# Alxaline/BraTS21

Hardware: AMD Instinct MI355X
Metric: train patches/sec (4x128^3, width-48) (higher is better)
Workload: dtype bf16; 1 GPU; equiunet width=48, batch=2/GPU of 4x128^3 synthetic patches, fwd + deep-supervision Dice + bwd + ranger (BASELINE.json configs[1]); global_batch=2, parallelism=dp1

## Files before the change

brats21_amd/csrc/conv_wgrad.hip:

```cpp
#include <stdlib.h>
#include "twin_begin.hpp"
#include "common.hpp"

typedef __attribute__((ext_vector_type(4))) short s16x4;

struct WgradParams {
  const void* x1; const void* x2; int c1, c2, p1, p2;
  const void* dy; int dyp;
  float* ws;
  int N, D, H, W, cin, cout;
  int tz, ty, tx, ntiles, nsplit;
  int nlane;
  int ntaps, dil;
  int seglen, nsegz;
};

constexpr int WG_TZ = 4, WG_TY = 4, WG_TX = 16, WG_VOX = 256;

template <typename T, int DIL, int COF, int CIF, int KS = 3>
struct WgGeom {
  static constexpr bool BF = std::is_same<T, bf16_t>::value;
  static constexpr int ESZ = sizeof(T);
  static constexpr int EPL = 16 / ESZ;
  static constexpr int R = KS == 3 ? DIL : 0;
  static constexpr int HY = WG_TY + 2 * R, HX = WG_TX + 2 * R;
  static constexpr int HVOX = WG_TZ * HY * HX;
  static constexpr int CI_T = 16 * CIF, CO_T = 16 * COF;
  static constexpr int XROWB = CI_T * ESZ, YROWB = CO_T * ESZ;
  static constexpr int SX = BF ? (CIF == 1 ? 32 : 96) : XROWB + 16;
  static constexpr int SY = BF ? (COF == 1 ? 32 : 96) : YROWB + 16;
  static constexpr int XPPV = XROWB / 16, YPPV = YROWB / 16;
  static constexpr int XPPR = HX * XPPV, XIPR = (XPPR + 63) / 64, XROWS = WG_TZ * HY, XRPW = (XROWS + 3) / 4;
  static constexpr int YPPR = WG_TX * YPPV, YIPR = (YPPR + 63) / 64, YROWS = WG_TZ * WG_TY, YRPW = YROWS / 4;
  static constexpr int LDS_X = HVOX * SX, LDS_Y = WG_VOX * SY;
  static constexpr int LDS = LDS_X + LDS_Y;
  static constexpr int PAIRS = (KS == 3 ? 9 : 1) * CIF;
  static constexpr int PPW = (PAIRS + 3) / 4;
  static constexpr int NB = BF ? 32 : 64;
};

DEVI bf16x8 tr_pair(const char* p0, const char* p1) {
  const s16x4 lo = __builtin_amdgcn_ds_read_tr16_b64_v4i16((__attribute__((address_space(3))) s16x4*)p0);
  const s16x4 hi = __builtin_amdgcn_ds_read_tr16_b64_v4i16((__attribute__((address_space(3))) s16x4*)p1);
  typedef __attribute__((ext_vector_type(8))) short s16x8;
  const s16x8 v = {lo[0], lo[1], lo[2], lo[3], hi[0], hi[1], hi[2], hi[3]};
  return __builtin_bit_cast(bf16x8, v);
}

template <typename T, int DIL, int COF, int CIF, int KS = 3>
__global__ __launch_bounds__(256, 2) void conv_wgrad_kernel(const WgradParams p) {
  using G = WgGeom<T, DIL, COF, CIF, KS>;
  extern __shared__ __attribute__((aligned(16))) char lds[];
  char* ldx = lds;
  char* ldy = lds + G::LDS_X;
  const int tid = threadIdx.x, lane = tid & 63;
  const int wave = __builtin_amdgcn_readfirstlane(tid >> 6);
  const int q = lane >> 4, v = lane & 15;
  const int NP = KS == 3 ? 3 : p.ntaps;
  const int lane8 = blockIdx.x % p.nlane, rr = blockIdx.x / p.nlane;
  const int tzg = rr % NP, gsub = rr / NP, g8 = gridDim.x / (NP * p.nlane);
  const int shz = (KS == 3 || p.ntaps == 1) ? 0 : (tzg / 9 - 1) * p.dil;
  const int shy = (KS == 3 || p.ntaps == 1) ? 0 : ((tzg / 3) % 3 - 1) * p.dil;
  const int shx = (KS == 3 || p.ntaps == 1) ? 0 : (tzg % 3 - 1) * p.dil;
  const int split = lane8 + p.nlane * gsub;
  const int tpx = (p.ntiles + p.nlane - 1) / p.nlane;
  const int tile_end = min(p.ntiles, (lane8 + 1) * tpx);
  const int cot = blockIdx.y, cit = blockIdx.z;
  const int co0 = cot * G::CO_T, ci0 = cit * G::CI_T;
  const T* xsrc;
  int xpitch;
  if (ci0 < p.c1) { xsrc = (const T*)p.x1 + ci0; xpitch = p.p1; }
  else { xsrc = (const T*)p.x2 + (ci0 - p.c1); xpitch = p.p2; }
  const int ci_lim = (ci0 < p.c1 ? p.c1 : p.c1 + p.c2) - ci0;
  const int co_lim = p.cout - co0;

  int xhx[G::XIPR], xlo[G::XIPR];
  int xvo[G::XRPW][G::XIPR];
#pragma unroll
  for (int j = 0; j < G::XIPR; ++j) {
    const int pc = lane + 64 * j;
    const int hx = pc / G::XPPV, part = pc % G::XPPV;
    const bool ok = pc < G::XPPR && part * G::EPL < ci_lim;
    xhx[j] = ok ? hx : -100000;
    xlo[j] = pc < G::XPPR ? wave * (G::HX * G::SX) + hx * G::SX + part * 16 : -1;
#pragma unroll
    for (int k = 0; k < G::XRPW; ++k) {
      const int row = wave + 4 * k;
      xvo[k][j] = (((row / G::HY) * p.H + row % G::HY) * p.W + hx) * xpitch * G::ESZ + part * 16;
    }
  }
  int yvx[G::YIPR], ylo[G::YIPR];
  int yvo[G::YRPW][G::YIPR];
#pragma unroll
  for (int j = 0; j < G::YIPR; ++j) {
    const int pc = lane + 64 * j;
    const int vx = pc / G::YPPV, part = pc % G::YPPV;
    const bool ok = pc < G::YPPR && part * G::EPL < co_lim;
    yvx[j] = ok ? vx : 100000;
    ylo[j] = pc < G::YPPR ? wave * (WG_TX * G::SY) + vx * G::SY + part * 16 : -1;
#pragma unroll
    for (int k = 0; k < G::YRPW; ++k) {
      const int row = wave + 4 * k;
      yvo[k][j] = (((row / WG_TY) * p.H + row % WG_TY) * p.W + vx) * p.dyp * G::ESZ + part * 16;
    }
  }
  const unsigned xsample_bytes = (unsigned)p.D * p.H * p.W * xpitch * G::ESZ;
  const unsigned ysample_bytes = (unsigned)p.D * p.H * p.W * p.dyp * G::ESZ;

  int poff[G::PPW];
#pragma unroll
  for (int jj = 0; jj < G::PPW; ++jj) {
    const int pid = wave + 4 * jj;
    const int t9 = pid / CIF, nn = pid % CIF;
    poff[jj] = pid < G::PAIRS ? (((t9 / 3) * G::R) * G::HX + (t9 % 3) * G::R) * G::SX + nn * G::NB : 0;
  }
  f32x4 acc[G::PPW][COF];
#pragma unroll
  for (int jj = 0; jj < G::PPW; ++jj)
#pragma unroll
    for (int m = 0; m < COF; ++m) acc[jj][m] = f32x4{0.f, 0.f, 0.f, 0.f};

  u32x4 rx[G::XRPW][G::XIPR], ry[G::YRPW][G::YIPR];
  auto issue_loads = [&](int tile) {
    int bt = tile;
    const int x0 = (bt % p.tx) * WG_TX; bt /= p.tx;
    const int y0 = (bt % p.ty) * WG_TY; bt /= p.ty;
    const int z0 = (bt % p.tz) * WG_TZ;
    const int n = bt / p.tz;
    const int gz0 = KS == 3 ? z0 + (tzg - 1) * DIL : z0 + shz;
    const int gy0 = KS == 3 ? y0 - DIL : y0 + shy, gx0 = KS == 3 ? x0 - DIL : x0 + shx;
    const size_t sample_vox = (size_t)n * p.D * p.H * p.W;
    const __amdgpu_buffer_rsrc_t xrs = __builtin_amdgcn_make_buffer_rsrc((void*)(xsrc + sample_vox * xpitch), (short)0,
                                                                          (int)xsample_bytes, 0x00020000);
    const __amdgpu_buffer_rsrc_t yrs = __builtin_amdgcn_make_buffer_rsrc((void*)((const T*)p.dy + sample_vox * p.dyp + co0),
                                                                          (short)0, (int)ysample_bytes, 0x00020000);
    const int xorg = ((gz0 * p.H + gy0) * p.W + gx0) * xpitch * G::ESZ;
    const int yorg = ((z0 * p.H + y0) * p.W + x0) * p.dyp * G::ESZ;
    bool xok[G::XIPR], yok[G::YIPR];
#pragma unroll
    for (int j = 0; j < G::XIPR; ++j) xok[j] = (unsigned)(gx0 + xhx[j]) < (unsigned)p.W;
#pragma unroll
    for (int j = 0; j < G::YIPR; ++j) yok[j] = x0 + yvx[j] < p.W;
#pragma unroll
    for (int k = 0; k < G::XRPW; ++k) {
      const int row = wave + 4 * k;
      const int gz = gz0 + row / G::HY, gy = gy0 + row % G::HY;
      const bool row_ok = row < G::XROWS && (unsigned)gz < (unsigned)p.D && (unsigned)gy < (unsigned)p.H;
#pragma unroll
      for (int j = 0; j < G::XIPR; ++j) {
        const int vo = (row_ok && xok[j]) ? xorg + xvo[k][j] : -1;
        rx[k][j] = __builtin_bit_cast(u32x4, __builtin_amdgcn_raw_buffer_load_b128(xrs, vo, 0, 0));
      }
    }
#pragma unroll
    for (int k = 0; k < G::YRPW; ++k) {
      const int row = wave + 4 * k;
      const bool row_ok = z0 + row / WG_TY < p.D && y0 + row % WG_TY < p.H;
#pragma unroll
      for (int j = 0; j < G::YIPR; ++j) {
        const int vo = (row_ok && yok[j]) ? yorg + yvo[k][j] : -1;
        ry[k][j] = __builtin_bit_cast(u32x4, __builtin_amdgcn_raw_buffer_load_b128(yrs, vo, 0, 0));
      }
    }
  };
  constexpr bool PREFETCH = !(G::BF && KS == 3 && DIL == 2 && COF * CIF == 9);
  const int tile_first = lane8 * tpx + gsub;
  if (PREFETCH && tile_first < tile_end) issue_loads(tile_first);
  for (int tile = tile_first; tile < tile_end; tile += g8) {
    if (!PREFETCH) issue_loads(tile);
    __syncthreads();
#pragma unroll
    for (int k = 0; k < G::XRPW; ++k) {
      if (wave + 4 * k < G::XROWS) {
#pragma unroll
        for (int j = 0; j < G::XIPR; ++j)
          if (xlo[j] >= 0) *(u32x4*)(ldx + xlo[j] + k * 4 * (G::HX * G::SX)) = rx[k][j];
      }
    }
#pragma unroll
    for (int k = 0; k < G::YRPW; ++k) {
#pragma unroll
      for (int j = 0; j < G::YIPR; ++j)
        if (ylo[j] >= 0) *(u32x4*)(ldy + ylo[j] + k * 4 * (WG_TX * G::SY)) = ry[k][j];
    }
    __syncthreads();
    if (PREFETCH && tile + g8 < tile_end) issue_loads(tile + g8);
    __builtin_amdgcn_sched_barrier(0);

    if constexpr (G::BF) {
      const int qq = v >> 2, pp = v & 3;
      const int ybase = (4 * q + qq) * G::SY + pp * 8;
      const int xbase = (4 * q + qq) * G::SX + pp * 8;
      constexpr int PD = 3;
      bf16x8 a[2][COF], b[PD + 1];
      auto read_a = [&](auto s_) {
        constexpr int s = s_;
        const int yoff = ybase + (32 * s) * G::SY;
#pragma unroll
        for (int m = 0; m < COF; ++m) a[s & 1][m] = tr_pair(ldy + yoff + m * 32, ldy + yoff + 16 * G::SY + m * 32);
      };
      auto read_b = [&](auto u_) {
        constexpr int u = u_;
        constexpr int s = u / G::PPW, jj = u % G::PPW;
        const int xoff = xbase + (((s >> 1) * G::HY + 2 * (s & 1)) * G::HX) * G::SX + poff[jj];
        b[u % (PD + 1)] = tr_pair(ldx + xoff, ldx + xoff + G::HX * G::SX);
      };
      constexpr int NU = 8 * G::PPW;
      read_a(std::integral_constant<int, 0>{});
      static_for<0, PD>([&](auto u_) { read_b(u_); });
      static_for<0, NU>([&](auto u_) {
        constexpr int u = u_;
        constexpr int s = u / G::PPW, jj = u % G::PPW;
        if constexpr (u + PD < NU) read_b(std::integral_constant<int, u + PD>{});
        if constexpr (jj == 0 && s + 1 < 8) read_a(std::integral_constant<int, s + 1>{});
        __builtin_amdgcn_sched_barrier(0);
#pragma unroll
        for (int m = 0; m < COF; ++m)
          acc[jj][m] = MFMA16_16x16x32(a[s & 1][m], b[u % (PD + 1)], acc[jj][m]);
        __builtin_amdgcn_sched_barrier(0);
      });
    } else {
#pragma unroll 2
      for (int s = 0; s < 64; ++s) {
        const int vx = 4 * s + q;
        const int z = vx >> 6, y = (vx >> 4) & 3, x = vx & 15;
        const int yoff = vx * G::SY + v * 4;
        const int xoff = ((z * G::HY + y) * G::HX + x) * G::SX + v * 4;
        float a[COF];
#pragma unroll
        for (int m = 0; m < COF; ++m) a[m] = *(const float*)(ldy + yoff + m * 64);
#pragma unroll
        for (int jj = 0; jj < G::PPW; ++jj) {
          const float b = *(const float*)(ldx + xoff + poff[jj]);
#pragma unroll
          for (int m = 0; m < COF; ++m) acc[jj][m] = __builtin_amdgcn_mfma_f32_16x16x4f32(a[m], b, acc[jj][m], 0, 0, 0);
        }
      }
    }
  }

#pragma unroll
  for (int jj = 0; jj < G::PPW; ++jj) {
    const int pid = wave + 4 * jj;
    if (pid < G::PAIRS) {
      const int t9 = pid / CIF, nn = pid % CIF;
      float* base = p.ws + (KS == 3 ? (size_t)split * 27 + tzg * 9 + t9 : (size_t)split * p.ntaps + tzg) * p.cout * p.cin;
      const int ci = ci0 + nn * 16 + v;
#pragma unroll
      for (int m = 0; m < COF; ++m)
#pragma unroll
        for (int r = 0; r < 4; ++r) {
          const int co = co0 + m * 16 + 4 * q + r;
          if (co < p.cout && nn * 16 + v < ci_lim) base[(size_t)co * p.cin + ci] = acc[jj][m][r];
        }
    }
  }
}

template <int CIF, int COF = 3> struct Wg3 {
  static constexpr int HZ = WG_TZ + 2, HY = WG_TY + 2, HX = WG_TX + 2, HVOX = HZ * HY * HX;
  static constexpr int CO = 16 * COF;
  static constexpr int SX = CIF == 3 ? 96 : 32, SY = COF == 3 ? 96 : 160, XPPV = 2 * CIF, YPPV = 2 * COF;
  static constexpr int XPIECES = HVOX * XPPV, YPIECES = WG_VOX * YPPV;
  static constexpr int XI = (XPIECES + 511) / 512, YI = YPIECES / 512;
  static constexpr int LDS_X = HVOX * SX, LDS = LDS_X + WG_VOX * SY;
  static constexpr int PAIRS = 27 * CIF, PPW = (PAIRS + 7) / 8;
};

template <int CIF, int COF = 3>
__global__ __launch_bounds__(512, 1) void conv_wgrad_alltaps_kernel(const WgradParams p) {
  typedef bf16_t T;
  using G = Wg3<CIF, COF>;
  static_assert(COF == 3 || CIF == 1, "four co fragments: the first-layer form only");
  extern __shared__ __attribute__((aligned(16))) char lds[];
  char* ldx = lds;
  char* ldy = lds + G::LDS_X;
  const int tid = threadIdx.x, lane = tid & 63;
  const int wave = __builtin_amdgcn_readfirstlane(tid >> 6);
  const int q = lane >> 4, v = lane & 15;
  const int lane8 = blockIdx.x % p.nlane, gsub = blockIdx.x / p.nlane, g8 = gridDim.x / p.nlane;
  const int split = blockIdx.x;
  const int tpx = (p.ntiles + p.nlane - 1) / p.nlane;
  const int tile_end = min(p.ntiles, (lane8 + 1) * tpx);
  const int co0 = blockIdx.y * G::CO, ci0 = blockIdx.z * 16 * CIF;
  const int ci_lim = (ci0 < p.c1 ? p.c1 : p.c1 + p.c2) - ci0;
  const T* xsrc;
  int xpitch;
  if (ci0 < p.c1) { xsrc = (const T*)p.x1 + ci0; xpitch = p.p1; }
  else { xsrc = (const T*)p.x2 + (ci0 - p.c1); xpitch = p.p2; }

  int xcode[G::XI], ycode[G::YI];
#pragma unroll
  for (int i = 0; i < G::XI; ++i) {
    const int P = tid + 512 * i;
    const int vox = P / G::XPPV, part = P % G::XPPV;
    const int hx = vox % G::HX, hy = (vox / G::HX) % G::HY, hz = vox / (G::HX * G::HY);
    xcode[i] = (P < G::XPIECES && part * 8 < ci_lim) ? (hz | hy << 3 | hx << 6 | part << 11 | 1 << 14) : 0;
  }
#pragma unroll
  for (int i = 0; i < G::YI; ++i) {
    const int P = tid + 512 * i;
    const int vox = P / G::YPPV, part = P % G::YPPV;
    ycode[i] = (vox >> 6) | ((vox >> 4) & 3) << 3 | (vox & 15) << 6 | part << 11 | 1 << 14;
  }
  const unsigned xsample_bytes = (unsigned)p.D * p.H * p.W * xpitch * 2;
  const unsigned ysample_bytes = (unsigned)p.D * p.H * p.W * p.dyp * 2;

  int poff[G::PPW];
#pragma unroll
  for (int jj = 0; jj < G::PPW; ++jj) {
    const int pid = wave + 8 * jj;
    const int t = pid / CIF, nn = pid % CIF;
    poff[jj] = pid < G::PAIRS ? (((t / 9) * G::HY + (t / 3) % 3) * G::HX + t % 3) * G::SX + nn * 32 : 0;
  }
  f32x4 acc[G::PPW][COF];
#pragma unroll
  for (int jj = 0; jj < G::PPW; ++jj)
#pragma unroll
    for (int m = 0; m < COF; ++m) acc[jj][m] = f32x4{0.f, 0.f, 0.f, 0.f};

  u32x4 rx[G::XI], ry[G::YI];
  auto issue_loads = [&](int tile) {
    int bt = tile;
    const int x0 = (bt % p.tx) * WG_TX; bt /= p.tx;
    const int y0 = (bt % p.ty) * WG_TY; bt /= p.ty;
    const int z0 = (bt % p.tz) * WG_TZ;
    const int n = bt / p.tz;
    const size_t sample_vox = (size_t)n * p.D * p.H * p.W;
    const __amdgpu_buffer_rsrc_t xrs = __builtin_amdgcn_make_buffer_rsrc((void*)(xsrc + sample_vox * xpitch), (short)0,
                                                                          (int)xsample_bytes, 0x00020000);
    const __amdgpu_buffer_rsrc_t yrs = __builtin_amdgcn_make_buffer_rsrc((void*)((const T*)p.dy + sample_vox * p.dyp + co0),
                                                                          (short)0, (int)ysample_bytes, 0x00020000);
    unsigned zm = 0, ym = 0, xm = 0, zy = 0, yy = 0, xy = 0;
#pragma unroll
    for (int h = 0; h < G::HZ; ++h) zm |= ((unsigned)(z0 - 1 + h) < (unsigned)p.D ? 1u : 0u) << h;
#pragma unroll
    for (int h = 0; h < G::HY; ++h) ym |= ((unsigned)(y0 - 1 + h) < (unsigned)p.H ? 1u : 0u) << h;
#pragma unroll
    for (int h = 0; h < G::HX; ++h) xm |= ((unsigned)(x0 - 1 + h) < (unsigned)p.W ? 1u : 0u) << h;
    zy = zm >> 1; yy = ym >> 1; xy = xm >> 1;
    const int xorg = ((z0 - 1) * p.H + (y0 - 1)) * p.W + (x0 - 1);
    const int yorg = (z0 * p.H + y0) * p.W + x0;
    const int xpb = xpitch * 2, ypb = p.dyp * 2;
#pragma unroll
    for (int i = 0; i < G::XI; ++i) {
      int c = xcode[i];
      asm volatile("" : "+v"(c));
      const unsigned ok = (unsigned)(c >> 14) & (zm >> (c & 7)) & (ym >> ((c >> 3) & 7)) & (xm >> ((c >> 6) & 31)) & 1u;
      const int pv = ((c & 7) * p.H + ((c >> 3) & 7)) * p.W + ((c >> 6) & 31);
      const int vo = ok ? (xorg + pv) * xpb + ((c >> 11) & 7) * 16 : -1;
      rx[i] = __builtin_bit_cast(u32x4, __builtin_amdgcn_raw_buffer_load_b128(xrs, vo, 0, 0));
    }
#pragma unroll
    for (int i = 0; i < G::YI; ++i) {
      int c = ycode[i];
      asm volatile("" : "+v"(c));
      const unsigned ok = (zy >> (c & 7)) & (yy >> ((c >> 3) & 7)) & (xy >> ((c >> 6) & 31)) & 1u;
      const int pv = ((c & 7) * p.H + ((c >> 3) & 7)) * p.W + ((c >> 6) & 31);
      const int vo = ok ? (yorg + pv) * ypb + ((c >> 11) & 7) * 16 : -1;
      ry[i] = __builtin_bit_cast(u32x4, __builtin_amdgcn_raw_buffer_load_b128(yrs, vo, 0, 0));
    }
  };

  const int tile_first = lane8 * tpx + gsub;
  if (tile_first < tile_end) issue_loads(tile_first);
  for (int tile = tile_first; tile < tile_end; tile += g8) {
    __syncthreads();
#pragma unroll
    for (int i = 0; i < G::XI; ++i)
      if (tid + 512 * i < G::XPIECES) *(u32x4*)(ldx + (tid + 512 * i) * 16) = rx[i];
#pragma unroll
    for (int i = 0; i < G::YI; ++i) {
      const int P = tid + 512 * i;
      *(u32x4*)(ldy + (P / G::YPPV) * G::SY + (P % G::YPPV) * 16) = ry[i];
    }
    __syncthreads();
    if (tile + g8 < tile_end) issue_loads(tile + g8);
    __builtin_amdgcn_sched_barrier(0);
// ... 506 lines not shown
  __syncthreads();
  const size_t pair0 = (size_t)blockIdx.x * 128, npairs = (size_t)cout * cin;
  float* dst = dw + pair0 * taps;
  const float isc = amax ? x3_inv_scale(x3_scale_from_amax(*amax)) : 1.f;
  for (int i = threadIdx.x; i < 128 * taps; i += blockDim.x) {
    const int pr = i / taps, tap = i % taps;
    if (pair0 + pr < npairs) dst[i] = red_tile[tap * 128 + pr] * isc;
  }
}

static void wgrad_reduce_launch(const float* ws, float* dw, int nsplit, int cout, int cin, int taps, hipStream_t st,
                                const float* amax = nullptr) {
  const size_t per = (size_t)taps * cout * cin;
  const size_t tblocks = ((size_t)cout * cin / 4 + 31) / 32;
  if (taps > 1 && taps <= 32 && tblocks >= 256)
    hipLaunchKernelGGL(wgrad_reduce_taps_kernel, dim3((unsigned)tblocks), dim3(256), (size_t)taps * 128 * sizeof(float), st, ws, dw,
                       nsplit, cout, cin, taps, amax);
  else
    hipLaunchKernelGGL(wgrad_reduce_kernel, dim3((unsigned)((per / 4 + 31) / 32)), dim3(256), 0, st, ws, dw, nsplit, cout, cin, taps, amax);
}

template <typename T>
__global__ void dbias_kernel(const T* __restrict__ dy, int pitch, float* __restrict__ db, size_t voxels, int C) {
  __shared__ float red[256];
  const int c = blockIdx.x;
  float s = 0.f;
  for (size_t v = threadIdx.x; v < voxels; v += blockDim.x) s += to_f<T>(dy[v * pitch + c]);
  red[threadIdx.x] = s;
  __syncthreads();
  for (int m = 128; m > 0; m >>= 1) {
    if ((int)threadIdx.x < m) red[threadIdx.x] += red[threadIdx.x + m];
    __syncthreads();
  }
  if (threadIdx.x == 0) db[c] = red[0];
}

static int wgrad_nlane(int ntiles) {
  int nl = 8;
  while (nl > 1 && ntiles / nl < 16) nl >>= 1;
  return nl;
}
static int wgrad_g8(int ntiles, int cotiles, int citiles) {
  const int nl = wgrad_nlane(ntiles);
  int g8 = ceil_div(512, 3 * nl * cotiles * citiles);
  const int cap = ceil_div(ntiles, nl);
  if (g8 > cap) g8 = cap;
  if (g8 < 1) g8 = 1;
  return g8;
}
static int wgrad_nsplit(int ntiles, int cotiles, int citiles) { return wgrad_nlane(ntiles) * wgrad_g8(ntiles, cotiles, citiles); }
static void wgrad_tiles(int dtype, int c1, int c2, int cout, int* cof, int* cif) {
  const int co16 = ceil_div(cout, 16);
  *cof = co16 % 3 == 0 ? 3 : (co16 % 2 == 0 ? 2 : 1);
  if (dtype == BRATS_F32) { *cif = 1; return; }
  const int a = ceil_div(c1, 16), b = c2 > 0 ? ceil_div(c2, 16) : 0;
  auto ok = [&](int f) { return a % f == 0 && (b == 0 || b % f == 0); };
  *cif = ok(3) ? 3 : (ok(2) ? 2 : 1);
}

int g_wgrad_alltaps_mode = -1;
static bool wgrad_alltaps_ok(int dtype, int dil, int c1, int c2, int cout, int ntiles, int* g8_out, int* wide_out = nullptr) {
  static int env_mode = -1, ncu = 0;
  if (env_mode < 0) {
    const char* e = getenv("BRATS_WGRAD_ALLTAPS");
    env_mode = e ? atoi(e) : 1;
    int dev = 0;
    hipDeviceProp_t prop;
    ncu = (hipGetDevice(&dev) == hipSuccess && hipGetDeviceProperties(&prop, dev) == hipSuccess) ? prop.multiProcessorCount : 256;
  }
  const int mode = g_wgrad_alltaps_mode >= 0 ? g_wgrad_alltaps_mode : env_mode;
  const int cin = c1 + (c2 > 0 ? c2 : 0);
  const bool narrow = c2 <= 0 && c1 <= 16;
  if (!mode || dtype != BRATS_BF16 || dil != 1) return false;
  bool wide = false;
  if (cout % 48 || (!narrow && (c1 % 48 || (c2 > 0 && c2 % 48)))) {
    if (cout % 64 || (!narrow && (c1 % 32 || (c2 > 0 && c2 % 32)))) return false;
    wide = true;
  }
  const int blocks = wide ? (cout / 64) * (narrow ? 1 : cin / 32) : (cout / 48) * (narrow ? 1 : cin / 48);
  const int nl = wgrad_nlane(ntiles);
  int g8 = ceil_div(ncu, nl * blocks);
  if (g8 < 1) g8 = 1;
  if (ntiles < 4 * nl * g8) return false;
  *g8_out = g8;
  if (wide_out) *wide_out = wide ? 1 : 0;
  return true;
}
extern "C" int BRATS_API(brats_conv3d_set_wgrad_alltaps)(int mode) {
  const int old = g_wgrad_alltaps_mode;
  g_wgrad_alltaps_mode = mode < 0 ? -1 : (mode ? 1 : 0);
  return old;
}

static size_t x3_align(size_t b);
static size_t wgrad_x3_fused_ws_bytes(int N, int D, int H, int W, int c1, int c2, int cout);
extern "C" size_t BRATS_API(brats_conv3d_wgrad_ws_bytes)(int dtype, int ksize, int N, int D, int H, int W, int c1, int c2, int cout) {
  if (ksize != 3) return 0;
  if (dtype == BRATS_X3_BF16) {
    const size_t vox = (size_t)N * D * H * W;
    const size_t slab = BRATS_API(brats_conv3d_wgrad_ws_bytes)(BRATS_BF16, 3, N, D, H, W, c1, c2, cout) * 3;
    auto sp = [&](int c) { return c > 0 ? 2 * x3_align(vox * c * 2) : (size_t)0; };
    const size_t three = x3_align(slab) + sp(c1) + sp(c2) + sp(cout), fused = wgrad_x3_fused_ws_bytes(N, D, H, W, c1, c2, cout);
    return three > fused ? three : fused;
  }
  int cof, cif;
  wgrad_tiles(dtype, c1, c2, cout, &cof, &cif);
  const int ntiles = N * ceil_div(D, WG_TZ) * ceil_div(H, WG_TY) * ceil_div(W, WG_TX);
  const int cin_tiles = ceil_div(c1, 16 * cif) + (c2 > 0 ? ceil_div(c2, 16 * cif) : 0);
  int ns = wgrad_nsplit(ntiles, ceil_div(cout, 16 * cof), cin_tiles);
  int g8 = 0;
  if (wgrad_alltaps_ok(dtype, 1, c1, c2, cout, ntiles, &g8) && wgrad_nlane(ntiles) * g8 > ns) ns = wgrad_nlane(ntiles) * g8;
  return (size_t)ns * 27 * cout * (c1 + (c2 > 0 ? c2 : 0)) * sizeof(float);
}

template <typename T, int DIL, int COF, int CIF, int KS = 3>
static int wgrad_launch(const WgradParams& p, dim3 grid, hipStream_t st) {
  using G = WgGeom<T, DIL, COF, CIF, KS>;
  auto kern = conv_wgrad_kernel<T, DIL, COF, CIF, KS>;
  static std::atomic<uint64_t> attr_done{0};
  BRATS_ENSURE_LDS_ATTR(kern, G::LDS, attr_done);
  hipLaunchKernelGGL(kern, grid, dim3(256), G::LDS, st, p);
  BRATS_CHECK_LAUNCH();
  return 0;
}

template <typename T, int DIL, int KS = 3>
static int wgrad_dispatch(const WgradParams& p, int cof, int cif, dim3 grid, hipStream_t st) {
#define WG_CASE(A, B) if (cof == A && cif == B) return wgrad_launch<T, DIL, A, B, KS>(p, grid, st);
  WG_CASE(3, 1) WG_CASE(2, 1) WG_CASE(1, 1)
  if constexpr (std::is_same<T, bf16_t>::value) {
    WG_CASE(3, 3) WG_CASE(3, 2) WG_CASE(2, 3) WG_CASE(2, 2) WG_CASE(1, 3) WG_CASE(1, 2)
  }
#undef WG_CASE
  BRATS_FAIL(BRATS_E_UNSUPPORTED, "wgrad: unsupported tile %dx%d", cof, cif);
}

static int wgrad_mfma(const void* x1, int c1, int pitch1, const void* x2, int c2, int pitch2, const void* dy, int dypitch, float* ws,
                      int dtype, int dil, int N, int D, int H, int W, int cout, hipStream_t st, int* nsplit_out) {
  int cof, cif;
  wgrad_tiles(dtype, c1, c2, cout, &cof, &cif);
  WgradParams p;
  p.x1 = x1; p.x2 = x2; p.c1 = c1; p.c2 = c2; p.p1 = pitch1; p.p2 = pitch2;
  p.dy = dy; p.dyp = dypitch; p.ws = ws;
  p.N = N; p.D = D; p.H = H; p.W = W; p.cin = c1 + c2; p.cout = cout;
  p.tz = ceil_div(D, WG_TZ); p.ty = ceil_div(H, WG_TY); p.tx = ceil_div(W, WG_TX);
  p.ntiles = N * p.tz * p.ty * p.tx;
  const int cot = ceil_div(cout, 16 * cof);
  const int cit = ceil_div(c1, 16 * cif) + (c2 > 0 ? ceil_div(c2, 16 * cif) : 0);
  p.nsplit = wgrad_nsplit(p.ntiles, cot, cit);
  p.nlane = wgrad_nlane(p.ntiles);
  if (c2 > 0 && c1 % (16 * cif)) BRATS_FAIL(BRATS_E_UNSUPPORTED, "wgrad: c1=%d must be a multiple of the ci tile %d", c1, 16 * cif);
  int g8a = 0, wide = 0;
  const bool alltaps = wgrad_alltaps_ok(dtype, dil, c1, c2, cout, p.ntiles, &g8a, &wide);
  if (!alltaps && ((c1 + c2) % 16 || cout % 16)) {
    hipError_t e = hipMemsetAsync(ws, 0, (size_t)p.nsplit * 27 * cout * p.cin * sizeof(float), st);
    if (e != hipSuccess) BRATS_FAIL(BRATS_E_HIP, "wgrad: memset: %s", hipGetErrorString(e));
  }
  dim3 grid(3 * p.nsplit, cot, cit);
  int rc;
  if (alltaps) {
    p.nsplit = p.nlane * g8a;
    constexpr int lds_48 = Wg3b<3, 3>::LDS, lds_wide = Wg3b<4, 2>::LDS;
    static std::atomic<uint64_t> attr_b{0}, attr_c{0}, attr_d{0}, attr_e{0};
    BRATS_ENSURE_LDS_ATTR(conv_wgrad_alltaps_kernel<1>, Wg3<1>::LDS, attr_b);
    BRATS_ENSURE_LDS_ATTR((conv_wgrad_alltaps_kernel<1, 4>), (Wg3<1, 4>::LDS), attr_e);
    BRATS_ENSURE_LDS_ATTR((conv_wgrad_alltaps2_kernel<3, 3>), lds_48, attr_c);
    BRATS_ENSURE_LDS_ATTR((conv_wgrad_alltaps2_kernel<4, 2>), lds_wide, attr_d);
    if (wide && c2 <= 0 && c1 <= 16) {
      hipLaunchKernelGGL((conv_wgrad_alltaps_kernel<1, 4>), dim3(p.nsplit, cout / 64, 1), dim3(512), (Wg3<1, 4>::LDS), st, p);
    } else if (wide) {
      hipLaunchKernelGGL((conv_wgrad_alltaps2_kernel<4, 2>), dim3(p.nsplit, cout / 64, p.cin / 32), dim3(512), lds_wide, st, p);
    } else if (c2 <= 0 && c1 <= 16 && c1 % 8 == 0) {
      static std::atomic<uint64_t> attr_f{0};
      BRATS_ENSURE_LDS_ATTR((conv_wgrad_alltaps2_kernel<3, 1>), (Wg3b<3, 1>::LDS), attr_f);
      hipLaunchKernelGGL((conv_wgrad_alltaps2_kernel<3, 1>), dim3(p.nsplit, cout / 48, 1), dim3(512), (Wg3b<3, 1>::LDS), st, p);
    } else if (c2 <= 0 && c1 <= 16) {
      hipLaunchKernelGGL(conv_wgrad_alltaps_kernel<1>, dim3(p.nsplit, cout / 48, 1), dim3(512), Wg3<1>::LDS, st, p);
    } else {
      hipLaunchKernelGGL((conv_wgrad_alltaps2_kernel<3, 3>), dim3(p.nsplit, cout / 48, p.cin / 48), dim3(512), lds_48, st, p);
    }
    rc = 0;
  } else if (dtype == BRATS_BF16) rc = dil == 1 ? wgrad_dispatch<bf16_t, 1>(p, cof, cif, grid, st) : wgrad_dispatch<bf16_t, 2>(p, cof, cif, grid, st);
  else rc = dil == 1 ? wgrad_dispatch<float, 1>(p, cof, cif, grid, st) : wgrad_dispatch<float, 2>(p, cof, cif, grid, st);
  if (rc) return rc;
  BRATS_CHECK_LAUNCH();
  *nsplit_out = p.nsplit;
  return 0;
}

template <int V>
__global__ void __launch_bounds__(256) x3_split_kernel(const float* __restrict__ src, int pitch, bf16_t* __restrict__ hi,
                                                       bf16_t* __restrict__ lo, size_t voxels, int C, const float* __restrict__ amax) {
  const float sc = amax ? x3_scale_from_amax(*amax) : 1.f;
  const int cv = C / 8;
  const size_t total = voxels * cv;
  const size_t stride = (size_t)gridDim.x * 256;
  auto load = [&](size_t i, u32x4& a, u32x4& b) {
    const float* p = src + (i / cv) * pitch + (i % cv) * 8;
    a = __builtin_nontemporal_load((const u32x4*)p);
    b = __builtin_nontemporal_load((const u32x4*)(p + 4));
  };
  auto emit = [&](size_t i, const u32x4& a, const u32x4& b) {
    const uint32_t w[8] = {a[0], a[1], a[2], a[3], b[0], b[1], b[2], b[3]};
    uint32_t h[4], l[4];
#pragma unroll
    for (int e = 0; e < 4; ++e) {
      const float x0 = __uint_as_float(w[2 * e]) * sc, x1 = __uint_as_float(w[2 * e + 1]) * sc;
      x3_split2(x0, x1, h[e], l[e]);
    }
    const size_t o = (i / cv) * C + (i % cv) * 8;
    __builtin_nontemporal_store(u32x4{h[0], h[1], h[2], h[3]}, (u32x4*)(hi + o));
    __builtin_nontemporal_store(u32x4{l[0], l[1], l[2], l[3]}, (u32x4*)(lo + o));
  };
  size_t i = (size_t)blockIdx.x * 256 + threadIdx.x;
  for (; i + stride < total; i += 2 * stride) {
    u32x4 a0, b0, a1, b1;
    load(i, a0, b0);
    load(i + stride, a1, b1);
    emit(i, a0, b0);
    emit(i + stride, a1, b1);
  }
  if (i < total) {
    u32x4 a0, b0;
    load(i, a0, b0);
    emit(i, a0, b0);
  }
}
static size_t x3_align(size_t b) { return (b + 255) / 256 * 256; }
static size_t wgrad_x3_split_bytes(size_t voxels, int c) { return c > 0 ? x3_align(voxels * c * 2) : 0; }
static void x3_split_launch(const float* src, int pitch, bf16_t* hi, bf16_t* lo, size_t vox, int c, const float* amax, hipStream_t st) {
  const size_t total = vox * (c / 8);
  size_t nb = (total + 511) / 512;
  const unsigned blocks = (unsigned)(nb < 1 ? 1 : (nb > 262144 ? 262144 : nb));
  hipLaunchKernelGGL(x3_split_kernel<0>, dim3(blocks), dim3(256), 0, st, src, pitch, hi, lo, vox, c, amax);
}

static int wgrad_x3(const void* x1, int c1, int pitch1, const void* x2, int c2, int pitch2, const void* dy, int dypitch,
                    const float* amax_dy, float* ws, float* dw, size_t slab_bytes, int dil, int N, int D, int H, int W, int cout,
                    hipStream_t st) {
  const size_t vox = (size_t)N * D * H * W;
  char* b = (char*)ws + x3_align(slab_bytes);
  bf16_t* h1 = (bf16_t*)b; b += wgrad_x3_split_bytes(vox, c1);
  bf16_t* l1 = (bf16_t*)b; b += wgrad_x3_split_bytes(vox, c1);
  bf16_t* h2 = (bf16_t*)b; b += wgrad_x3_split_bytes(vox, c2);
  bf16_t* l2 = (bf16_t*)b; b += wgrad_x3_split_bytes(vox, c2);
  bf16_t* hy = (bf16_t*)b; b += wgrad_x3_split_bytes(vox, cout);
  bf16_t* ly = (bf16_t*)b;
  auto split = [&](const void* src, int pitch, bf16_t* hi, bf16_t* lo, int c, const float* amax) {
    x3_split_launch((const float*)src, pitch, hi, lo, vox, c, amax, st);
  };
  split(x1, pitch1, h1, l1, c1, nullptr);
  if (c2 > 0) split(x2, pitch2, h2, l2, c2, nullptr);
  split(dy, dypitch, hy, ly, cout, amax_dy);
  BRATS_CHECK_LAUNCH();
  int ns = 0, total = 0;
  const size_t per = (size_t)27 * cout * (c1 + c2);
  int rc = wgrad_mfma(l1, c1, c1, c2 > 0 ? l2 : nullptr, c2, c2, hy, cout, ws, BRATS_BF16, dil, N, D, H, W, cout, st, &ns);
  if (rc) return rc;
  total += ns;
  rc = wgrad_mfma(h1, c1, c1, c2 > 0 ? h2 : nullptr, c2, c2, ly, cout, ws + (size_t)total * per, BRATS_BF16, dil, N, D, H, W, cout, st, &ns);
  if (rc) return rc;
  total += ns;
  rc = wgrad_mfma(h1, c1, c1, c2 > 0 ? h2 : nullptr, c2, c2, hy, cout, ws + (size_t)total * per, BRATS_BF16, dil, N, D, H, W, cout, st, &ns);
  if (rc) return rc;
  total += ns;
  wgrad_reduce_launch((const float*)ws, dw, total, cout, c1 + c2, 27, st, amax_dy);
  return 0;
}

#include "conv_wgrad_x3.hpp"
extern "C" int BRATS_API(brats_conv3d_set_x3_wgrad_fused)(int mode) {
  const int old = g_x3_wgrad_fused_mode;
  g_x3_wgrad_fused_mode = mode < 0 ? -1 : (mode > 2 ? 2 : mode);
  return old;
}

static int wgrad_impl(const void* x1, int c1, int pitch1, const void* x2, int c2, int pitch2, const void* dy, int dypitch,
                      const float* amax_dy, float* ws, float* dw, float* dbias, int dtype, int ksize, int dil, int N, int D, int H,
                      int W, int cout, brats_stream_t s) {
  if (!x1 || !dy || !ws || !dw || c1 <= 0 || cout <= 0) BRATS_FAIL(BRATS_E_ARG, "wgrad: null pointer / bad size");
  if (ksize != 3 || (dil != 1 && dil != 2)) BRATS_FAIL(BRATS_E_UNSUPPORTED, "wgrad: ksize=%d dil=%d unsupported", ksize, dil);
  if (c2 < 0) c2 = 0;
  if (c2 > 0 && !x2) BRATS_FAIL(BRATS_E_ARG, "wgrad: c2 > 0 but x2 NULL");
  const bool x3 = dtype == BRATS_X3_BF16;
  const int epl = dtype == BRATS_BF16 ? 8 : 4;
  if (pitch1 % epl || (c2 && pitch2 % epl) || dypitch % epl || c1 % epl || c2 % epl || cout % epl)
    BRATS_FAIL(BRATS_E_ARG, "wgrad: channel counts / pitches must be multiples of %d", epl);
  if (x3 && (c1 % 8 || c2 % 8 || cout % 8)) BRATS_FAIL(BRATS_E_ARG, "wgrad (split precision): channel counts must be multiples of 8");
  {
    const int mp = pitch1 > pitch2 ? (pitch1 > dypitch ? pitch1 : dypitch) : (pitch2 > dypitch ? pitch2 : dypitch);
    if ((double)D * H * W * mp * (dtype == BRATS_BF16 ? 2 : 4) >= 2147483648.0)
      BRATS_FAIL(BRATS_E_UNSUPPORTED, "wgrad: one sample of %dx%dx%d x pitch %d exceeds the 2 GiB buffer-offset range", D, H, W, mp);
  }
  hipStream_t st = (hipStream_t)s;
  if (x3) {
    int rc = wgrad_x3_fused(x1, c1, pitch1, x2, c2, pitch2, dy, dypitch, amax_dy, ws, dw, dil, N, D, H, W, cout, st);
    if (rc == 1) {
      const size_t slab = BRATS_API(brats_conv3d_wgrad_ws_bytes)(BRATS_BF16, 3, N, D, H, W, c1, c2, cout) * 3;
      rc = wgrad_x3(x1, c1, pitch1, x2, c2, pitch2, dy, dypitch, amax_dy, ws, dw, slab, dil, N, D, H, W, cout, st);
    }
    if (rc) return rc;
  } else {
    int nsplit = 0;
    const int rc = wgrad_mfma(x1, c1, pitch1, x2, c2, pitch2, dy, dypitch, ws, dtype, dil, N, D, H, W, cout, st, &nsplit);
    if (rc) return rc;
    wgrad_reduce_launch((const float*)ws, dw, nsplit, cout, c1 + c2, 27, st);
// ... 211 lines not shown
```

Before: 139.8 patches/s.

## Reshape dilated bf16 wgrad tile to 2x8x16 and resize split grid

For bf16 dilation-2 3x3x3 weight-gradient convs, the voxel tile changes from 4x4x16 to 2x8x16. With fewer z-planes the halo is smaller, so less LDS and fewer x-loads are needed per tile. The launcher recomputes the tile counts, lane count and split factor for this path, capped by the workspace split count. Occupancy is now stated per CU through a computed workgroups-per-CU bound with static asserts on LDS fit. The y-halo grows, and the split grid changes how the reduction work is spread.

```diff
diff --git a/brats21_amd/csrc/conv_wgrad.hip b/brats21_amd/csrc/conv_wgrad.hip
--- a/brats21_amd/csrc/conv_wgrad.hip
+++ b/brats21_amd/csrc/conv_wgrad.hip
@@ -16,6 +16,7 @@
 };
 
 constexpr int WG_TZ = 4, WG_TY = 4, WG_TX = 16, WG_VOX = 256;
+constexpr int WG_CU_LDS = 160 * 1024;
 
 template <typename T, int DIL, int COF, int CIF, int KS = 3>
 struct WgGeom {
@@ -23,17 +24,23 @@
   static constexpr int ESZ = sizeof(T);
   static constexpr int EPL = 16 / ESZ;
   static constexpr int R = KS == 3 ? DIL : 0;
-  static constexpr int HY = WG_TY + 2 * R, HX = WG_TX + 2 * R;
-  static constexpr int HVOX = WG_TZ * HY * HX;
+  static constexpr bool FLAT = BF && KS == 3 && DIL == 2;
+  static constexpr int TZ = FLAT ? 2 : WG_TZ, TY = FLAT ? 8 : WG_TY;
+  static_assert(TZ * TY * WG_TX == WG_VOX && TY % 2 == 0, "256 voxels; a k-step is two x-rows of one z-plane");
+  static constexpr int HY = TY + 2 * R, HX = WG_TX + 2 * R;
+  static constexpr int HVOX = TZ * HY * HX;
   static constexpr int CI_T = 16 * CIF, CO_T = 16 * COF;
   static constexpr int XROWB = CI_T * ESZ, YROWB = CO_T * ESZ;
   static constexpr int SX = BF ? (CIF == 1 ? 32 : 96) : XROWB + 16;
   static constexpr int SY = BF ? (COF == 1 ? 32 : 96) : YROWB + 16;
   static constexpr int XPPV = XROWB / 16, YPPV = YROWB / 16;
-  static constexpr int XPPR = HX * XPPV, XIPR = (XPPR + 63) / 64, XROWS = WG_TZ * HY, XRPW = (XROWS + 3) / 4;
-  static constexpr int YPPR = WG_TX * YPPV, YIPR = (YPPR + 63) / 64, YROWS = WG_TZ * WG_TY, YRPW = YROWS / 4;
+  static constexpr int XPPR = HX * XPPV, XIPR = (XPPR + 63) / 64, XROWS = TZ * HY, XRPW = (XROWS + 3) / 4;
+  static constexpr int YPPR = WG_TX * YPPV, YIPR = (YPPR + 63) / 64, YROWS = TZ * TY, YRPW = YROWS / 4;
   static constexpr int LDS_X = HVOX * SX, LDS_Y = WG_VOX * SY;
   static constexpr int LDS = LDS_X + LDS_Y;
+  static constexpr int WPC = 2 * LDS <= WG_CU_LDS ? 2 : 1;
+  static_assert(WPC * LDS <= WG_CU_LDS, "the tiles of the promised workgroups per CU must fit its LDS");
+  static_assert(!BF || WPC == 2, "every 16-bit form is built for two workgroups per CU");
   static constexpr int PAIRS = (KS == 3 ? 9 : 1) * CIF;
   static constexpr int PPW = (PAIRS + 3) / 4;
   static constexpr int NB = BF ? 32 : 64;
@@ -48,7 +55,7 @@
 }
 
 template <typename T, int DIL, int COF, int CIF, int KS = 3>
-__global__ __launch_bounds__(256, 2) void conv_wgrad_kernel(const WgradParams p) {
+__global__ __launch_bounds__(256, (WgGeom<T, DIL, COF, CIF, KS>::WPC)) void conv_wgrad_kernel(const WgradParams p) {
   using G = WgGeom<T, DIL, COF, CIF, KS>;
   extern __shared__ __attribute__((aligned(16))) char lds[];
   char* ldx = lds;
@@ -101,7 +108,7 @@
 #pragma unroll
     for (int k = 0; k < G::YRPW; ++k) {
       const int row = wave + 4 * k;
-      yvo[k][j] = (((row / WG_TY) * p.H + row % WG_TY) * p.W + vx) * p.dyp * G::ESZ + part * 16;
+      yvo[k][j] = (((row / G::TY) * p.H + row % G::TY) * p.W + vx) * p.dyp * G::ESZ + part * 16;
     }
   }
   const unsigned xsample_bytes = (unsigned)p.D * p.H * p.W * xpitch * G::ESZ;
@@ -124,8 +131,8 @@
   auto issue_loads = [&](int tile) {
     int bt = tile;
     const int x0 = (bt % p.tx) * WG_TX; bt /= p.tx;
-    const int y0 = (bt % p.ty) * WG_TY; bt /= p.ty;
-    const int z0 = (bt % p.tz) * WG_TZ;
+    const int y0 = (bt % p.ty) * G::TY; bt /= p.ty;
+    const int z0 = (bt % p.tz) * G::TZ;
     const int n = bt / p.tz;
     const int gz0 = KS == 3 ? z0 + (tzg - 1) * DIL : z0 + shz;
     const int gy0 = KS == 3 ? y0 - DIL : y0 + shy, gx0 = KS == 3 ? x0 - DIL : x0 + shx;
@@ -155,7 +162,7 @@
 #pragma unroll
     for (int k = 0; k < G::YRPW; ++k) {
       const int row = wave + 4 * k;
-      const bool row_ok = z0 + row / WG_TY < p.D && y0 + row % WG_TY < p.H;
+      const bool row_ok = z0 + row / G::TY < p.D && y0 + row % G::TY < p.H;
 #pragma unroll
       for (int j = 0; j < G::YIPR; ++j) {
         const int vo = (row_ok && yok[j]) ? yorg + yvo[k][j] : -1;
@@ -202,7 +209,7 @@
       auto read_b = [&](auto u_) {
         constexpr int u = u_;
         constexpr int s = u / G::PPW, jj = u % G::PPW;
-        const int xoff = xbase + (((s >> 1) * G::HY + 2 * (s & 1)) * G::HX) * G::SX + poff[jj];
+        const int xoff = xbase + ((((2 * s) / G::TY) * G::HY + (2 * s) % G::TY) * G::HX) * G::SX + poff[jj];
         b[u % (PD + 1)] = tr_pair(ldx + xoff, ldx + xoff + G::HX * G::SX);
       };
       constexpr int NU = 8 * G::PPW;
@@ -223,7 +230,7 @@
 #pragma unroll 2
       for (int s = 0; s < 64; ++s) {
         const int vx = 4 * s + q;
-        const int z = vx >> 6, y = (vx >> 4) & 3, x = vx & 15;
+        const int z = (vx >> 4) / G::TY, y = (vx >> 4) % G::TY, x = vx & 15;
         const int yoff = vx * G::SY + v * 4;
         const int xoff = ((z * G::HY + y) * G::HX + x) * G::SX + v * 4;
         float a[COF];
@@ -1036,6 +1043,20 @@
   if (c2 > 0 && c1 % (16 * cif)) BRATS_FAIL(BRATS_E_UNSUPPORTED, "wgrad: c1=%d must be a multiple of the ci tile %d", c1, 16 * cif);
   int g8a = 0, wide = 0;
   const bool alltaps = wgrad_alltaps_ok(dtype, dil, c1, c2, cout, p.ntiles, &g8a, &wide);
+  if (!alltaps && dtype == BRATS_BF16 && dil == 2) {
+    using GF = WgGeom<bf16_t, 2, 3, 3>;
+    const int ns_ws = p.nsplit;
+    p.tz = ceil_div(D, GF::TZ); p.ty = ceil_div(H, GF::TY);
+    p.ntiles = N * p.tz * p.ty * p.tx;
+    p.nlane = wgrad_nlane(p.ntiles);
+    while (p.nlane > ns_ws) p.nlane >>= 1;
+    int g8 = ceil_div(512, 3 * p.nlane * cot * cit);
+    const int cap = ceil_div(p.ntiles, p.nlane);
+    if (g8 > cap) g8 = cap;
+    if (g8 > ns_ws / p.nlane) g8 = ns_ws / p.nlane;
+    if (g8 < 1) g8 = 1;
+    p.nsplit = p.nlane * g8;
+  }
   if (!alltaps && ((c1 + c2) % 16 || cout % 16)) {
     hipError_t e = hipMemsetAsync(ws, 0, (size_t)p.nsplit * 27 * cout * p.cin * sizeof(float), st);
     if (e != hipSuccess) BRATS_FAIL(BRATS_E_HIP, "wgrad: memset: %s", hipGetErrorString(e));
```

Result: no change. 139.5 patches/s (-0.2%).
